# dkotfis/Octree-SLAM

Hardware: AMD Instinct MI355X
Metric: SLAM frames/sec (fuse+ICP+raycast) (higher is better)
Workload: dtype u32/f32 (ICP sums exact fixed-point in f64); 1 GPU; cfg3: synthetic 640x480 RGB-D stream, depth-12 SVO, half-edge 4.096 m, bilateral+ICP(19 it)+fuse+raycast(reference mode); parallelism=single GPU, frames_in_map_at_end=300, frames_input=resident in HBM

## Files before the change

### include/svoslam.h

```cpp
#ifndef SVOSLAM_H_
#define SVOSLAM_H_

#include <stddef.h>
#include <stdint.h>

#ifdef __cplusplus
extern "C" {
#endif

#define SVOSLAM_ABI_VERSION 1

typedef enum {
  SVOSLAM_OK = 0,
  SVOSLAM_ERR_INVALID_ARG = -1,
  SVOSLAM_ERR_NO_DEVICE = -2,
  SVOSLAM_ERR_HIP = -3,
  SVOSLAM_ERR_OOM = -4,
  SVOSLAM_ERR_DEPTH = -5,
  SVOSLAM_ERR_POOL_LIMIT = -6,
  SVOSLAM_ERR_TRACKING_LOST = -7,
  SVOSLAM_ERR_IO = -8,
  SVOSLAM_ERR_FORMAT = -9
} svoslam_status;

#define SVOSLAM_MAX_DEPTH 16
#define SVOSLAM_FLAG_CHILDREN 0x40000000u
#define SVOSLAM_CHILD_MASK 0x3FFFFFFFu

int svoslam_abi_version(void);
const char *svoslam_status_string(int status);

typedef struct svoslam_config {
  int32_t march_bricks;
  int32_t track_mode;
  int32_t track_workers;
  int32_t track_stream;
  int32_t runner_deferred;
  int32_t runner_lead;
  int32_t runner_prio;
  int32_t runner_replicas;
  int32_t runner_timeline;
  int32_t sort_pairs;
  int32_t graphs;
  int32_t march_ahead;
  int32_t reserved[4];
} svoslam_config;
int svoslam_config_get(svoslam_config *out);
int svoslam_config_set(const svoslam_config *in);
const char *svoslam_last_error(void);
const char *svoslam_device_arch(void);

typedef struct {
  uint32_t *d_data;
  int32_t size;
  int32_t capacity;
  int32_t *d_size;
  int32_t pending;
  int64_t pending_bound;
  void *tracker;
} svoslam_pool;

int svoslam_pool_init(svoslam_pool *pool, int32_t capacity_nodes, void *stream);
int svoslam_pool_reserve(svoslam_pool *pool, int32_t capacity_nodes, void *stream);
int svoslam_pool_free(svoslam_pool *pool);
int svoslam_pool_reset(svoslam_pool *pool, void *stream);
int svoslam_pool_sync(svoslam_pool *pool, void *stream);
int svoslam_pool_expand(svoslam_pool *pool, float center[3], float *edge_length, const float toward[3], void *stream);
int svoslam_pool_save(svoslam_pool *pool, const char *path, const float center[3], float edge_length, int32_t max_depth,
                      void *stream);
int svoslam_pool_touch(svoslam_pool *pool);
int svoslam_pool_march_accel(const svoslam_pool *pool, int32_t *has_grid, int32_t *brick_state, int32_t *brick_shift);
int svoslam_pool_set_nodes(svoslam_pool *pool, const uint32_t *h_words, int32_t num_nodes, void *stream);
int svoslam_pool_evict_subtree(svoslam_pool *pool, const uint8_t *path, int32_t levels, const char *file, void *stream);
int svoslam_pool_restore_subtree(svoslam_pool *pool, const char *file, void *stream);
int svoslam_subtree_file_nodes(const char *file, uint32_t **h_words, int32_t *num_nodes);
int svoslam_pool_graft_subtree(svoslam_pool *pool, const char *file, void *stream);
typedef struct {
  int32_t size_before, size_after;
  int32_t capacity_before, capacity_after;
  int32_t levels;
  int32_t tiles_dropped;
} svoslam_compact_stats;
int svoslam_pool_compact(svoslam_pool *pool, int32_t capacity_nodes, uint32_t *d_old_tile, svoslam_compact_stats *stats,
                         void *stream);
int svoslam_pool_copy(svoslam_pool *dst, svoslam_pool *src, void *stream);
int svoslam_pool_load(svoslam_pool *pool, const char *path, float center[3], float *edge_length, int32_t *max_depth,
                      void *stream);

typedef struct svoslam_workspace svoslam_workspace;
int svoslam_workspace_create(svoslam_workspace **ws);
int svoslam_workspace_destroy(svoslam_workspace *ws);

typedef struct {
  int32_t num_points;
  int32_t num_split;
  int32_t pass_sizes[SVOSLAM_MAX_DEPTH + 1];
  int32_t pool_size_before;
  int32_t pool_size_after;
} svoslam_fuse_stats;

int svoslam_svo_from_point_cloud(svoslam_workspace *ws, const float *d_points, const uint8_t *d_colors,
                                 int32_t n, int32_t max_depth, svoslam_pool *pool, const float center[3],
                                 float edge_length, svoslam_fuse_stats *stats, void *stream);

int svoslam_svo_from_point_cloud_async(svoslam_workspace *ws, const float *d_points, const uint8_t *d_colors,
                                       int32_t n, int32_t max_depth, svoslam_pool *pool, const float center[3],
                                       float edge_length, void *stream);

int svoslam_svo_fuse_sort(svoslam_workspace *ws, const float *d_points, int32_t n, int32_t max_depth,
                          const float center[3], float edge_length, void *stream);
int svoslam_svo_fuse_sort_frame(svoslam_workspace *ws, const uint16_t *d_depth, const float *d_pose, int32_t width, int32_t height,
                                float fx, float fy, int32_t max_depth, const float center[3], float edge_length, float *d_bbox7,
                                void *stream);
int svoslam_svo_fuse_plan(svoslam_workspace *ws, int32_t n, int32_t max_depth, svoslam_pool *pool, void *stream);
// ... 252 lines not shown
```

### octree-slam_amd/__init__.py

```python
import ctypes as C
import os

import numpy as np

_HERE = os.path.dirname(os.path.abspath(__file__))
LIB_PATH = os.path.join(_HERE, "libsvoslam_hip.so")
HEADER_PATH = os.path.join(os.path.dirname(_HERE), "include", "svoslam.h")

MAX_DEPTH = 16
FLAG_CHILDREN = 0x40000000
CHILD_MASK = 0x3FFFFFFF
RENDER_REFERENCE = 0
RENDER_CARRY = 1
PYRAMID_ITERS = (10, 5, 4)
DELTA_FLOATS = 20


class SvoslamError(RuntimeError):
    pass


def build(verbose=False, force=False):
    import importlib.util
    spec = importlib.util.spec_from_file_location("_svoslam_build", os.path.join(_HERE, "build.py"))
# ... 67 lines not shown
    "svoslam_svo_fuse_split_early": (C.c_int, [_vp, _i32, _i32, C.POINTER(_PoolStruct), _vp]),
    "svoslam_svo_fuse_plan_structure": (C.c_int, [_vp, _i32, _i32, C.POINTER(_PoolStruct), _vp]),
    "svoslam_svo_fuse_adopt_sorted": (C.c_int, [_vp, _vp, _vp, _i32, _i32]),
    "svoslam_svo_fuse_sort_frame_band": (C.c_int, [_vp, _vp, _vp, _i32, _i32, _f32, _f32, _i32, _fp, _f32, _i32, _i32, _vp]),
    "svoslam_svo_fuse_merge_sorted": (C.c_int, [C.POINTER(_vp), C.POINTER(_vp), C.POINTER(_i32), _i32, _vp, _vp, _vp]),
    "svoslam_svo_fuse_export_sorted": (C.c_int, [_vp, _i32, _vp, _vp, _vp]),
    "svoslam_pool_structure_begin": (C.c_int, [C.POINTER(_PoolStruct), _vp]),
    "svoslam_svo_fuse_commit_deferred": (C.c_int, [_vp, _vp, _i32, _i32, C.POINTER(_PoolStruct), _vp]),
    "svoslam_svo_fuse_apply": (C.c_int, [_vp, C.POINTER(_PoolStruct), _vp]),
    "svoslam_svo_fuse_keyrange_commit": (C.c_int, [_vp, _vp, _vp, _vp, _i32, _i32, C.POINTER(_PoolStruct), _i32, _i32, _vp, C.c_int64, _vp]),
    "svoslam_svo_fuse_keyrange_apply": (C.c_int, [_vp, _vp, _i32, _i32, C.POINTER(_PoolStruct), C.POINTER(C.c_void_p), _i32, _vp]),
    "svoslam_svo_fuse_keyrange_status": (C.c_int, [_vp, C.POINTER(C.c_int32), _vp]),
    "svoslam_svo_fuse_keyrange_discard": (C.c_int, [_vp, C.POINTER(_PoolStruct)]),
    "svoslam_frame_reader_open": (C.c_int, [C.POINTER(_vp), C.c_char_p, _f32]),
    "svoslam_frame_reader_close": (C.c_int, [_vp]),
    "svoslam_frame_reader_info": (C.c_int, [_vp, C.POINTER(_i32), C.POINTER(_i32), C.POINTER(_i32)]),
    "svoslam_frame_reader_rewind": (C.c_int, [_vp]),
    "svoslam_frame_reader_next_host": (C.c_int, [_vp, _vp, _vp, C.POINTER(C.c_longlong), C.POINTER(_i32)]),
    "svoslam_frame_reader_next": (C.c_int, [_vp, _vp, _vp, C.POINTER(C.c_longlong), C.POINTER(_i32), _vp]),
    "svoslam_focal_from_fov": (C.c_int, [_i32, _i32, _f32, _f32, _fp, _fp]),
    "svoslam_image_load": (C.c_int, [C.c_char_p, C.POINTER(_vp), C.POINTER(_i32), C.POINTER(_i32), C.POINTER(_i32), C.POINTER(_i32)]),
    "svoslam_workspace_create": (C.c_int, [C.POINTER(_vp)]),
    "svoslam_workspace_destroy": (C.c_int, [_vp]),
    "svoslam_svo_from_point_cloud": (C.c_int, [_vp, _vp, _vp, _i32, _i32, C.POINTER(_PoolStruct), _fp, _f32,
                                                C.POINTER(FuseStats), _vp]),
    "svoslam_svo_from_voxel_grid": (C.c_int, [_vp, _vp, _vp, _i32, _i32, C.POINTER(_PoolStruct), _fp, _f32,
                                               C.POINTER(FuseStats), _vp]),
    "svoslam_extract_voxel_grid": (C.c_int, [_vp, C.POINTER(_PoolStruct), _i32, _fp, _f32, C.POINTER(_vp),
                                              C.POINTER(_vp), C.POINTER(_i32), _vp]),
    "svoslam_mesh_load_obj": (C.c_int, [C.c_char_p, C.POINTER(MeshStruct)]),
    "svoslam_mesh_free": (C.c_int, [C.POINTER(MeshStruct)]),
    "svoslam_texture_load_bmp": (C.c_int, [C.c_char_p, C.POINTER(TextureStruct)]),
    "svoslam_texture_free": (C.c_int, [C.POINTER(TextureStruct)]),
    "svoslam_mesh_to_voxel_grid": (C.c_int, [_vp, C.POINTER(MeshStruct), C.POINTER(TextureStruct), _i32, _i32, C.POINTER(_vp),
                                             C.POINTER(_vp), C.POINTER(_vp), C.POINTER(_i32), _fp, _vp]),
    "svoslam_mesh_last_fragments": (C.c_int, [_vp, C.POINTER(C.c_int64)]),
    "svoslam_voxel_grid_to_mesh": (C.c_int, [_vp, _vp, _vp, _i32, _f32, _fp, _i32, C.POINTER(C.c_int32), _i32, _fp, _vp, _vp, _vp, _vp, _vp]),
    "svoslam_memcpy_h2d": (C.c_int, [_vp, _vp, C.c_size_t]),
    "svoslam_memcpy_d2h": (C.c_int, [_vp, _vp, C.c_size_t]),
    "svoslam_runner_run_model": (C.c_int, [_vp, C.POINTER(_vp), C.POINTER(_vp), C.POINTER(C.c_longlong), _fp, _i32, _vp, _i32, _i32, _vp,
                                           _f32, C.POINTER(_i32), _vp]),
    "svoslam_runner_create": (C.c_int, [C.POINTER(_vp), _vp, C.POINTER(_PoolStruct), _i32, _i32, _i32, _fp, _f32, _f32, _f32, _i32]),
    "svoslam_runner_destroy": (C.c_int, [_vp]),
    "svoslam_runner_timeline": (C.c_int, [_vp, _fp, _i32, C.POINTER(_i32)]),
    "svoslam_runner_run": (C.c_int, [_vp, C.POINTER(_vp), C.POINTER(_vp), C.POINTER(C.c_longlong), _fp, _i32, _vp, _i32, _i32, _vp, _vp]),
    "svoslam_runner_bbox": (C.c_int, [_vp, _fp]),
# ... 122 lines not shown


def _stream():
    global _raw_stream
    import torch
    if _raw_stream is None:
        _raw_stream = getattr(torch._C, "_cuda_getCurrentRawStream", None) or False
    if _raw_stream:
        return C.c_void_p(_raw_stream(torch.cuda.current_device()))
    return C.c_void_p(torch.cuda.current_stream().cuda_stream)


def _ptr(t):
    return C.c_void_p(t.data_ptr()) if t is not None else C.c_void_p(0)


def _fa(values, n):
    a = (C.c_float * n)(*[float(v) for v in np.asarray(values, dtype=np.float32).reshape(-1)])
    return a


class ConfigStruct(C.Structure):
    _fields_ = [(n, C.c_int32) for n in ("march_bricks", "track_mode", "track_workers", "track_stream", "runner_deferred", "runner_lead",
                                         "runner_prio", "runner_replicas", "runner_timeline", "sort_pairs", "graphs", "march_ahead")] + [("reserved", C.c_int32 * 4)]


def get_config():
    c = ConfigStruct()
    check(lib().svoslam_config_get(C.byref(c)))
    return {n: int(getattr(c, n)) for n, _ in ConfigStruct._fields_ if n != "reserved"}


def configure(**settings):
    c = ConfigStruct()
    check(lib().svoslam_config_get(C.byref(c)))
    before = {n: int(getattr(c, n)) for n, _ in ConfigStruct._fields_ if n != "reserved"}
    for k, v in settings.items():
        if k not in before:
            raise KeyError("svoslam_config has no field %r" % (k,))
        setattr(c, k, int(v))
    check(lib().svoslam_config_set(C.byref(c)))
    return before


def config_env(**settings):
    return {"SVOSLAM_CONFIG": ",".join("%s=%d" % (k, int(v)) for k, v in settings.items())}


def device_arch():
    a = lib().svoslam_device_arch()
    return a.decode() if a else None


class Workspace:
    def __init__(self):
        self._h = C.c_void_p()
        check(lib().svoslam_workspace_create(C.byref(self._h)))

    def close(self):
        if self._h:
            lib().svoslam_workspace_destroy(self._h)
            self._h = C.c_void_p()

    def __del__(self):
        try:
            self.close()
        except Exception:
            pass


class Pool:

    def __init__(self, capacity_nodes=8):
        self._p = _PoolStruct(None, 0, 0, None, 0, 0)
        check(lib().svoslam_pool_init(C.byref(self._p), capacity_nodes, _stream()))

    @property
    def size(self):
        if self._p.pending > 0:
            check(lib().svoslam_pool_sync(C.byref(self._p), _stream()))
        return int(self._p.size)

    @property
    def capacity(self):
        return int(self._p.capacity)
# ... 932 lines not shown
```

### octree-slam_amd/csrc/abi.hip

```cpp
#include <stdarg.h>
#include <stdio.h>
#include <string.h>

#include "common.hpp"
#include "cone_trace.hpp"
#include "icp.hpp"
#include "image_kernels.hpp"
#include "map_query.hpp"
#include "mesh.hpp"
#include "model_depth.hpp"
#include "frame_io.hpp"
#include "pool_grid.hpp"
#include "stage_timing.hpp"
#include "svo_build.hpp"
#include "workspace.hpp"

namespace svoslam {

static thread_local char g_last_error[512] = "";
static char g_arch[256] = "";
static int g_device_state = 0;

void set_last_error_text(const char *fmt, ...) {
  va_list ap;
// ... 279 lines not shown
  void *p = malloc(img.data.size() ? img.data.size() : 1);
  if (!p) return SVOSLAM_ERR_OOM;
  memcpy(p, img.data.data(), img.data.size());
  *h_data = p;
  if (width) *width = img.width;
  if (height) *height = img.height;
  if (channels) *channels = img.channels;
  if (bits) *bits = img.bits;
  return SVOSLAM_OK;
}

int svoslam_workspace_create(svoslam_workspace **ws) {
  if (!ws) return SVOSLAM_ERR_INVALID_ARG;
  NEED_DEVICE();
  *ws = new svoslam_workspace();
  return SVOSLAM_OK;
}
int svoslam_workspace_destroy(svoslam_workspace *ws) {
  if (!ws) return SVOSLAM_OK;
  ws->release_all();
  delete ws;
  return SVOSLAM_OK;
}

int svoslam_svo_from_point_cloud(svoslam_workspace *ws, const float *d_points, const uint8_t *d_colors, int32_t n,
                                 int32_t max_depth, svoslam_pool *pool, const float center[3], float edge_length,
                                 svoslam_fuse_stats *stats, void *stream) {
  NEED_DEVICE();
  if (!center) return SVOSLAM_ERR_INVALID_ARG;
  return svo_from_point_cloud(ws, d_points, d_colors, n, max_depth, pool, center, edge_length, stats, S(stream));
}

int svoslam_svo_from_voxel_grid(svoslam_workspace *ws, const float *d_centers, const float *d_colors, int32_t n,
                                int32_t max_depth, svoslam_pool *pool, const float center[3], float edge_length,
                                svoslam_fuse_stats *stats, void *stream) {
  NEED_DEVICE();
  if (!center) return SVOSLAM_ERR_INVALID_ARG;
  return svo_from_voxel_grid(ws, d_centers, d_colors, n, max_depth, pool, center, edge_length, stats, S(stream));
}

int svoslam_extract_voxel_grid(svoslam_workspace *ws, const svoslam_pool *pool, int32_t max_depth, const float center[3],
                               float edge_length, float **d_centers, float **d_colors, int32_t *n_out, void *stream) {
  NEED_DEVICE();
  if (!center) return SVOSLAM_ERR_INVALID_ARG;
  return extract_voxel_grid(ws, pool, max_depth, center, edge_length, d_centers, d_colors, n_out, S(stream));
}
// ... 311 lines not shown
```

### octree-slam_amd/csrc/config.hip

```cpp
#include <cstdio>
#include <cstdlib>
#include <cstring>
#include <mutex>

#include "config.hpp"

namespace svoslam {
namespace {
std::mutex g_mu;
bool g_ready = false;
svoslam_config g_cfg;

struct Field { const char *name; int32_t svoslam_config::*member; };
const Field kFields[] = {
    {"march_bricks", &svoslam_config::march_bricks}, {"track_mode", &svoslam_config::track_mode},
    {"track_workers", &svoslam_config::track_workers}, {"track_stream", &svoslam_config::track_stream},
    {"runner_deferred", &svoslam_config::runner_deferred}, {"runner_lead", &svoslam_config::runner_lead},
    {"runner_prio", &svoslam_config::runner_prio}, {"runner_replicas", &svoslam_config::runner_replicas},
    {"runner_timeline", &svoslam_config::runner_timeline}, {"sort_pairs", &svoslam_config::sort_pairs},
    {"graphs", &svoslam_config::graphs}, {"march_ahead", &svoslam_config::march_ahead},
};

bool config_valid(const svoslam_config &c) {
  if (c.runner_replicas != 1 || c.graphs != 0) return false;
  if (c.track_mode < 0 || c.track_mode > 2 || c.track_workers < 0) return false;
  return true;
}

void init_locked() {
  if (g_ready) return;
  memset(&g_cfg, 0, sizeof(g_cfg));
  g_cfg.march_bricks = 1; g_cfg.track_stream = 1; g_cfg.march_ahead = 60;
  g_cfg.runner_deferred = -1; g_cfg.runner_lead = -1; g_cfg.runner_prio = -1; g_cfg.runner_replicas = 1;
  if (const char *e = getenv("SVOSLAM_CONFIG")) {
    const char *p = e;
    while (*p) {
      const char *eq = strchr(p, '='), *end = strchr(p, ',');
      if (!end) end = p + strlen(p);
      bool known = false;
      if (eq && eq < end && eq > p) {
        for (const Field &f : kFields)
          if ((size_t)(eq - p) == strlen(f.name) && strncmp(p, f.name, (size_t)(eq - p)) == 0) {
            known = true;
            svoslam_config trial = g_cfg;
            char *stop = nullptr;
            const long v = strtol(eq + 1, &stop, 10);
            trial.*(f.member) = (int32_t)v;
            if (stop == eq + 1 || stop != end || !config_valid(trial))
              fprintf(stderr, "svoslam: SVOSLAM_CONFIG: value of '%s' rejected (\"%.*s\"); the default stays\n", f.name, (int)(end - p), p);
            else
              g_cfg = trial;
          }
      }
      if (!known && end > p) fprintf(stderr, "svoslam: SVOSLAM_CONFIG: unknown or malformed entry \"%.*s\" ignored\n", (int)(end - p), p);
      p = *end ? end + 1 : end;
// ... 29 lines not shown
```

### octree-slam_amd/csrc/svo_build.hip

```cpp
#include <stdlib.h>
#include <string.h>

#include <cstdio>
#include <vector>

#include "radix_sort.hpp"
#include "image_device.hpp"
#include "config.hpp"
#include "pool_grid.hpp"
#include "svo_build.hpp"
#include "svo_fuse_internal.hpp"
#include "stage_timing.hpp"
#include "wave_rank.hpp"

namespace svoslam {

constexpr unsigned char kNotHead = 0xFE;
constexpr unsigned char kNoSplit = 0xFF;

template <int STRIDE>
__global__ __launch_bounds__(256) void compute_keys_kernel(const float *__restrict__ pts, int n, int depth, float cx,
                                                           float cy, float cz, float edge, u64 *__restrict__ keys, int idx_bits = -1) {
  const int i = blockIdx.x * 256 + threadIdx.x;
  if (i >= n) return;
// ... 463 lines not shown
__device__ inline void shadow_store(unsigned long long *__restrict__ shadow, u32 epoch, u32 node, u32 word) {
  shadow[node] = ((unsigned long long)epoch << 32) | word;
}

__global__ __launch_bounds__(256) void mip_level_kernel(int n, int d, const unsigned char *__restrict__ leaf_c,
                                                        const u32 *__restrict__ path_nodes, u32 *__restrict__ pool) {
  const long long j0 = ((long long)blockIdx.x * 256 + threadIdx.x) * 4;
  if (j0 >= n) return;
  u32 c4 = 0xFFFFFFFFu;
  if (j0 + 3 < n) c4 = *reinterpret_cast<const u32 *>(leaf_c + j0);
  else for (int k = 0; k < 4 && j0 + k < n; k++) c4 = (c4 & ~(0xFFu << (8 * k))) | ((u32)leaf_c[j0 + k] << (8 * k));
#pragma unroll
  for (int k = 0; k < 4; k++) {
    if ((int)((c4 >> (8 * k)) & 0xFFu) >= d) continue;
    const u32 node = path_nodes[(size_t)(d - 1) * n + (size_t)(j0 + k)];
    pool[2 * (size_t)node + 1] = average_tile(pool, pool[2 * (size_t)node] & kMask);
  }
}

__global__ void mip_root_kernel(u32 *__restrict__ pool, const PlanCounts *__restrict__ counts) {
  if (threadIdx.x == 0 && blockIdx.x == 0 && counts->any_valid) pool[1] = average_tile(pool, 0);
}

template <int MAXD>
__global__ __launch_bounds__(kFillThreads) void fill_mip_local_kernel(const u64 *__restrict__ skey, const u32 *__restrict__ sidx, int n,
                                                             int depth, const unsigned char *__restrict__ leaf_t,
                                                             const unsigned char *__restrict__ colors, u32 *__restrict__ pool,
                                                             u32 *__restrict__ strad, int num_tiles, u32 *__restrict__ grid_dirty,
                                                             unsigned long long *__restrict__ shadow, u32 epoch,
                                                             u32 *__restrict__ apply_nodes, const u64 *__restrict__ rec_key,
                                                             const u32 *__restrict__ bucket_base, const u32 *__restrict__ n0_saved,
                                                             const u32 *__restrict__ leaf_rec0, const u32 *__restrict__ leaf_start,
                                                             int *__restrict__ strad_bc, int brick_shift, const int *__restrict__ n_live) {
  if (n_live) { const int nl = *n_live; n = nl < n ? nl : n; }
  const bool early_links = leaf_rec0 != nullptr;
  SVO_HIGH_PRIO();
  __shared__ int last_owner[SVOSLAM_MAX_DEPTH + 1];
  __shared__ int next_pos, next_c;
  __shared__ int min_c;
  __shared__ u32 apply_cnt;
  const int tid = (int)threadIdx.x;
  const int bid = xcd_tile(num_tiles);
  if (bid >= num_tiles) return;
  int search_tiles = num_tiles;
  if (n_live) {
    const int live_tiles = (n + kFillThreads - 1) / kFillThreads;
    if (bid >= live_tiles) {
      if (tid >= 1 && tid < depth) {
        strad[2 * ((size_t)tid * num_tiles + bid)] = kNoStraddler;
        strad[2 * ((size_t)tid * num_tiles + bid) + 1] = 0u;
      }
      if (shadow && tid == 0) apply_nodes[(size_t)num_tiles * kFillThreads * (size_t)depth + bid] = 0u;
      return;
    }
    search_tiles = live_tiles;
  }
  if (tid == 0) apply_cnt = 0;
  u32 *apply_mine = apply_nodes ? apply_nodes + (size_t)bid * kFillThreads * (size_t)depth : nullptr;
  auto apply_append = [&](bool mine, u32 node) {
    const unsigned long long m = __ballot(mine);
    if (!m) return;
    u32 base = 0;
    if ((tid & 63) == 0) base = atomicAdd(&apply_cnt, (u32)__popcll(m));
    base = (u32)__shfl((int)base, 0);
    if (mine) apply_mine[base + (u32)__popcll(m & lanemask_lt())] = node;
  };
  const int j = bid * kFillThreads + tid;
  const int jn = j + kFillThreads;
  const unsigned char lt = j < n ? leaf_t[j] : kNotHead;
  const unsigned char ltn = jn < n ? leaf_t[jn] : kNotHead;
  const u64 key_j = j < n ? skey[j] : 1ull, key_p = (j > 0 && j < n) ? skey[j - 1] : 1ull;
  const u64 key_n = jn < n ? skey[jn] : 1ull, key_np = jn < n ? skey[jn - 1] : 1ull;
  const u32 point = j < n ? sidx[j] : 0u;
  const bool head = lt != kNotHead;
  const u32 start_base = (leaf_start && head) ? leaf_start[j] : 0u;
  u32 rec0 = 0;
  if (early_links && head && lt != kNoSplit) {
    const int cc = (key_p == 1ull) ? 0 : common_levels(key_j, key_p, depth);
    if (cc < (int)lt) rec0 = leaf_rec0[j];
  }
  u64 key = 1; int c = 0;
  if (head) { key = key_j; c = (key_p == 1ull) ? 0 : common_levels(key_j, key_p, depth); }
  if (grid_dirty && head && c < kPoolGridBlockLevel) pool_grid_mark(grid_dirty, key, depth);
  __shared__ u32 brick_cnt, brick_base;
  const bool bricks_on = grid_dirty != nullptr && brick_shift >= 0 && depth >= brick_node_level(brick_shift);
  u32 brick_entry = 0, brick_off = 0;
  const bool brick_mine = bricks_on && brick_mark_test(grid_dirty, head && c < brick_node_level(brick_shift), key, depth, brick_shift, brick_entry);
  if (tid <= SVOSLAM_MAX_DEPTH) {
    last_owner[tid] = -1;
    if (tid >= 1 && tid < depth) {
      strad[2 * ((size_t)tid * num_tiles + bid)] = kNoStraddler;
      strad[2 * ((size_t)tid * num_tiles + bid) + 1] = 0u;
    }
  }
  if (tid == 0) { next_pos = 0x7FFFFFFF; next_c = -1; min_c = 99; brick_cnt = 0u; }
  __syncthreads();
  if (bricks_on) {
    const unsigned long long bm = __ballot(brick_mine);
    if (bm) {
      const int leader = __ffsll((long long)bm) - 1;
      u32 woff = 0;
      if ((tid & 63) == leader) woff = atomicAdd(&brick_cnt, (u32)__popcll(bm));
      brick_off = (u32)__shfl((int)woff, leader) + (u32)__popcll(bm & ((1ull << (tid & 63)) - 1ull));
    }
  }
  if (head) {
    for (int d = c + 1; d < depth; d++) atomicMax(&last_owner[d], j);
    if (strad_bc) atomicMin(&min_c, c);
  }
  if (ltn != kNotHead) atomicMin(&next_pos, jn);
  __syncthreads();
  if (bricks_on && tid == 0 && brick_cnt) brick_base = brick_ring_reserve(grid_dirty, brick_cnt);
  if (next_pos == 0x7FFFFFFF) {
    for (int nb = bid + 2; nb < search_tiles; nb++) {
      const int jj = nb * kFillThreads + tid;
      if (jj < n && leaf_t[jj] != kNotHead) atomicMin(&next_pos, jj);
      __syncthreads();
      const bool found = next_pos != 0x7FFFFFFF;
      __syncthreads();
      if (found) break;
    }
    if (tid == 0 && next_pos != 0x7FFFFFFF) {
      u64 k2; int c2 = 0;
      (void)is_head(skey, next_pos, k2, c2, depth);
      next_c = c2;
    }
  } else if (jn == next_pos) {
    next_c = (key_np == 1ull) ? 0 : common_levels(key_n, key_np, depth);
  }
  if (strad_bc) {
    __syncthreads();
    if (tid == 0) { strad_bc[2 * bid] = next_c; strad_bc[2 * bid + 1] = min_c; }
  }
  int frontier = 0;
  int link_level = 0;
  u32 frontier_child = 0;
  bool have_rec0 = false;
  if (early_links) {
    __shared__ u32 wave_rec0[kFillThreads / 64];
    __shared__ int wave_has[kFillThreads / 64];
    const bool towner = head && lt != kNoSplit && c < (int)lt;
    const unsigned lane = (unsigned)tid & 63u, wv = (unsigned)tid >> 6;
    const unsigned long long om = __ballot(towner);
    const unsigned long long upto = om & ((lane == 63u) ? ~0ull : ((2ull << lane) - 1ull));
    const int src = upto ? 63 - __clzll((long long)upto) : -1;
    const u32 got = (u32)__shfl((int)rec0, src >= 0 ? src : 0);
    const int last = om ? 63 - __clzll((long long)om) : 0;
    const u32 lastv = (u32)__shfl((int)rec0, last);
    if (lane == 0) { wave_has[wv] = om != 0ull; wave_rec0[wv] = lastv; }
    __syncthreads();
    if (src >= 0) { rec0 = got; have_rec0 = true; }
    else {
      for (int w = (int)wv - 1; w >= 0; w--)
        if (wave_has[w]) { rec0 = wave_rec0[w]; have_rec0 = true; break; }
    }
// ... 24 lines not shown
  if (head) {
    const unsigned char *v = colors + 3 * (size_t)point;
    const unsigned char cr = v[0], cg = v[1], cb = v[2];
    int skip = 0;
    u32 base = 0, node = 0;
    if (leaf_start) {
      const int tt = lt == kNoSplit ? depth : (int)lt - 1;
      skip = c < tt ? c : tt;
      base = start_base;
    }
#pragma unroll
    for (int lvl = 1; lvl <= MAXD; lvl++) {
      if (lvl <= depth && lvl > skip) {
        node = base + ((u32)(key >> (3 * (depth - lvl))) & 7u);
        if (lvl == link_level) pool[2 * (size_t)node] = kFlag + (frontier_child & kMask);
        if (lvl < depth) {
          base = pool[2 * (size_t)node] & kMask;
          if (lvl == frontier) base = frontier_child & kMask;
          node_at[lvl] = node;
          child_at[lvl] = base;
        }
      }
    }
    const u32 word = blend_color256(pool[2 * (size_t)node + 1], cr, cg, cb);
    if (shadow) shadow_store(shadow, epoch, node, word);
    else pool[2 * (size_t)node + 1] = word;
    node_at[0] = node;
  }
  if (shadow) apply_append(head, node_at[0]);
  __syncthreads();
  if (brick_mine) brick_ring_store(grid_dirty, brick_base + brick_off, brick_entry);
#pragma unroll
  for (int d = MAXD - 1; d >= 1; d--) {
    if (d < depth) {
      u32 wrote = kNoStraddler;
      if (head && c < d) {
        if (j != last_owner[d] || next_c < d) {
          if (shadow) {
            shadow_store(shadow, epoch, node_at[d], average_tile_deferred(pool, shadow, epoch, child_at[d]));
            wrote = node_at[d];
          } else {
            pool[2 * (size_t)node_at[d] + 1] = average_tile(pool, child_at[d]);
          }
        } else {
          strad[2 * ((size_t)d * num_tiles + bid)] = node_at[d];
          strad[2 * ((size_t)d * num_tiles + bid) + 1] = child_at[d];
        }
      }
      if (shadow) apply_append(wrote != kNoStraddler, wrote);
      __syncthreads();
    }
  }
  if (brick_mine && lt != kNoSplit && (int)lt < brick_node_level(brick_shift)) brick_sibling_list(grid_dirty, brick_entry);
  if (shadow && tid == 0) apply_nodes[(size_t)num_tiles * kFillThreads * (size_t)depth + bid] = apply_cnt;
}

constexpr int kStradThreads = 1024;
__global__ __launch_bounds__(kStradThreads) void mip_straddle_kernel(u32 *__restrict__ pool, const u32 *__restrict__ strad, int num_tiles,
                                                            int depth, const PlanCounts *__restrict__ counts,
                                                            int *__restrict__ d_size, u32 *__restrict__ grid_dirty,
                                                            int32_t *__restrict__ h_sizes, int *__restrict__ d_slot,
                                                            unsigned long long *__restrict__ shadow, u32 epoch, int keep_size,
                                                            const int *__restrict__ n_live) {
  SVO_HIGH_PRIO();
  const int list_stride = num_tiles;
  if (n_live) { const int live = (*n_live + kFillThreads - 1) / kFillThreads; num_tiles = live < num_tiles ? live : num_tiles; }
  auto average = [&](u32 child_base) { return shadow ? average_tile_deferred(pool, shadow, epoch, child_base) : average_tile(pool, child_base); };
  auto store = [&](u32 node, u32 word) {
    if (shadow) shadow_store(shadow, epoch, node, word);
    else pool[2 * (size_t)node + 1] = word;
  };
  constexpr int kSlots = 8;
  const uint2 *list = reinterpret_cast<const uint2 *>(strad);
  const bool fits = num_tiles <= kSlots * kStradThreads;
  uint2 cur[kSlots], nxt[kSlots];
  auto fetch = [&](int d, uint2 *e) {
#pragma unroll
// ... 14 lines not shown
    } else {
      for (int t = (int)threadIdx.x; t < num_tiles; t += kStradThreads) {
        const uint2 e = list[(size_t)d * list_stride + t];
        if (e.x != kNoStraddler) store(e.x, average(e.y));
      }
    }
    __syncthreads();
  }
  if (threadIdx.x == 0) {
    if (counts->any_valid) store(0u, average(0u));
    if (!keep_size) {
      const int size_now = *d_size + 8 * counts->total_records;
      *d_size = size_now;
      if (h_sizes) {
        const int sl = *d_slot;
        h_sizes[sl] = size_now;
        *d_slot = (sl + 1) % 8;
      }
    }
  }
  if (grid_dirty) pool_grid_compact(grid_dirty, kStradThreads);
}

constexpr int kStradGroup = 16;
constexpr int kStrad2Threads = 256;
__global__ __launch_bounds__(kStrad2Threads) void mip_straddle2_kernel(u32 *__restrict__ pool, const u32 *__restrict__ strad,
                                                              const int *__restrict__ strad_bc, u32 *__restrict__ sstrad,
                                                              unsigned *__restrict__ ticket, int num_tiles, int depth,
                                                              const PlanCounts *__restrict__ counts, int *__restrict__ d_size,
                                                              u32 *__restrict__ grid_dirty, int32_t *__restrict__ h_sizes,
                                                              int *__restrict__ d_slot) {
  SVO_HIGH_PRIO();
  __shared__ int bc[kStradGroup], mc[kStradGroup];
  __shared__ int is_last;
  const int tid = (int)threadIdx.x, g = (int)blockIdx.x, groups = (int)gridDim.x;
  const int t0 = g * kStradGroup, t1 = (t0 + kStradGroup < num_tiles) ? t0 + kStradGroup : num_tiles;
  const uint2 *list = reinterpret_cast<const uint2 *>(strad);
  uint2 *super = reinterpret_cast<uint2 *>(sstrad);
  if (tid < kStradGroup) {
    bc[tid] = (t0 + tid < t1) ? strad_bc[2 * (t0 + tid)] : -1;
    mc[tid] = (t0 + tid < t1) ? strad_bc[2 * (t0 + tid) + 1] : 99;
  }
  __syncthreads();
  const int t = t0 + tid;
  for (int d = depth - 1; d >= 1; d--) {
    if (tid < kStradGroup) {
      uint2 sup = make_uint2(kNoStraddler, 0u);
// ... 469 lines not shown
    return SVOSLAM_OK;
  }
  const int64_t rmax = max_records(n, depth);
  if (pool != ws->planned_pool) {
    SVO_TRY(ensure_device_size(pool, stream));
    if ((int64_t)pool->size + pool->pending_bound + 8 * rmax > pool->capacity) {
      SVO_TRY(tracker_poll(pool, true));
      if ((int64_t)pool->size + pool->pending_bound + 8 * rmax > pool->capacity) return SVOSLAM_ERR_POOL_LIMIT;
    }
    pool->pending_bound += 8 * rmax;
  }
  const u64 *skey = ws->sorted_keys;
  const u32 *sidx = ws->sorted_idx;
  const unsigned char *leaf_t = ws->leaf_t.as<unsigned char>();
  int split_blocks = (int)cdiv(rmax, 256);
  if (split_blocks > 2048) split_blocks = 2048;
  const int fill_tiles = (int)cdiv(n, kFillThreads);
  const int strad_groups = (int)cdiv(fill_tiles, kStradGroup);
  const size_t strad_words = (size_t)(SVOSLAM_MAX_DEPTH + 1) * (size_t)fill_tiles * 2, bc_words = 2 * (size_t)fill_tiles;
  SVO_TRY(ws->strad.reserve((strad_words + bc_words + (size_t)(SVOSLAM_MAX_DEPTH + 1) * (size_t)strad_groups * 2) * 4));
  u32 *strad = ws->strad.as<u32>();
  int *strad_bc = reinterpret_cast<int *>(strad + strad_words);
  u32 *sstrad = strad + strad_words + bc_words;
  const bool two_tier = !deferred;
  const u32 *leaf_start = ws->leaf_start.as<u32>();
  SVO_TRY(ensure_device_size(pool, stream));
  PoolTracker *trk = tracker_of(pool);
  unsigned long long *shadow = nullptr;
  u32 epoch = 0, *apply_nodes = nullptr;
  if (deferred) {
    SVO_TRY(ws->apply_nodes.reserve(((size_t)fill_tiles * kFillThreads * (size_t)depth + (size_t)fill_tiles) * 4));
    apply_nodes = ws->apply_nodes.as<u32>();
    SVO_TRY(pool_shadow_begin(pool, stream, &shadow, &epoch));
    ws->deferred_pool = pool; ws->deferred_n = n; ws->deferred_depth = depth; ws->deferred_tiles = fill_tiles;
  }
  SVO_TRY(tracker_make_room(pool));
  int brick_shift = -1;
  u32 *grid_dirty = keyrange ? nullptr : pool_accel_dirty_bitmap(pool, deferred ? (int)(epoch & 1u) : 0, depth, &brick_shift);
  {
    StageScope timed(kStageFuseCommit, stream);
    if (!early)
      split_all_kernel<<<split_blocks, 256, 0, stream>>>(ws->rec_key.as<u64>(), ws->rec_front.as<u32>(),
                                                         ws->rec_pass.as<unsigned char>(), small_bucket_base(ws), small_counts(ws),
                                                         pool->d_data, pool->d_size, depth, grid_dirty, deferred ? small_n0(ws) : nullptr, 0);
    if (depth <= 12) fill_mip_local_kernel<12><<<xcd_grid(fill_tiles), kFillThreads, 0, stream>>>(skey, sidx, n, depth, leaf_t, d_colors, pool->d_data, strad, fill_tiles,
                                                                   grid_dirty, shadow, epoch, apply_nodes, ws->rec_key.as<u64>(),
                                                                   small_bucket_base(ws), small_n0(ws), early ? ws->leaf_rec0.as<u32>() : nullptr, leaf_start,
                                                                   two_tier ? strad_bc : nullptr, brick_shift, n_live);
    else fill_mip_local_kernel<16><<<xcd_grid(fill_tiles), kFillThreads, 0, stream>>>(skey, sidx, n, depth, leaf_t, d_colors, pool->d_data, strad, fill_tiles,
                                                                   grid_dirty, shadow, epoch, apply_nodes, ws->rec_key.as<u64>(),
                                                                   small_bucket_base(ws), small_n0(ws), early ? ws->leaf_rec0.as<u32>() : nullptr, leaf_start,
                                                                   two_tier ? strad_bc : nullptr, brick_shift, n_live);
    if (two_tier)
      mip_straddle2_kernel<<<strad_groups, kStrad2Threads, 0, stream>>>(pool->d_data, strad, strad_bc, sstrad, small_strad_ticket(ws), fill_tiles,
                                                                        depth, small_counts(ws), pool->d_size, grid_dirty,
                                                                        trk ? trk->h_size : nullptr, trk ? trk->d_slot : nullptr);
    else
      mip_straddle_kernel<<<1, kStradThreads, 0, stream>>>(pool->d_data, strad, fill_tiles, depth, small_counts(ws), pool->d_size, grid_dirty,
                                                           trk ? trk->h_size : nullptr, trk ? trk->d_slot : nullptr, shadow, epoch, keyrange ? 1 : 0, n_live);
    SVO_LAUNCH_CHECK();
  }
  if (keyrange) { ws->keyrange_bound = 8 * rmax; return SVOSLAM_OK; }
  pool->pending += 1;
  return tracker_push(pool, 8 * rmax, stream);
}

int svo_fuse_commit(svoslam_workspace *ws, const uint8_t *d_colors, int n, int depth, svoslam_pool *pool, hipStream_t stream) {
  return commit_impl(ws, d_colors, n, depth, pool, false, stream);
}

int svo_fuse_commit_deferred(svoslam_workspace *ws, const uint8_t *d_colors, int n, int depth, svoslam_pool *pool, hipStream_t stream) {
  return commit_impl(ws, d_colors, n, depth, pool, true, stream);
}

int svo_fuse_apply(svoslam_workspace *ws, svoslam_pool *pool, hipStream_t stream) {
  if (!ws || !pool || ws->deferred_pool != pool) return SVOSLAM_ERR_INVALID_ARG;
  ws->deferred_pool = nullptr;
  const int n = ws->deferred_n, depth = ws->deferred_depth, tiles = ws->deferred_tiles;
  if (n == 0) return SVOSLAM_OK;
  unsigned long long *shadow = nullptr;
  u32 epoch = 0;
  SVO_TRY(pool_shadow_current(pool, &shadow, &epoch));
// ... 57 lines not shown
```

### octree-slam_amd/csrc/workspace.hpp

```cpp
#pragma once

#include "common.hpp"

namespace svoslam {

struct DeviceBuffer {
  void *ptr = nullptr;
  size_t bytes = 0;
  int reserve(size_t need) {
    if (need <= bytes) return SVOSLAM_OK;
    if (ptr) { SVO_HIP(hipFree(ptr)); ptr = nullptr; bytes = 0; }
    size_t want = need + need / 4 + 256;
    SVO_HIP(hipMalloc(&ptr, want));
    bytes = want;
    return SVOSLAM_OK;
  }
  void release() {
    if (ptr) (void)hipFree(ptr);
    ptr = nullptr; bytes = 0;
  }
  template <class T> T *as() const { return reinterpret_cast<T *>(ptr); }
};

struct PlanCounts {
  int32_t total_records;
  int32_t pass_start[SVOSLAM_MAX_DEPTH + 2];
  int32_t any_valid;
};

}

struct svoslam_workspace {
  svoslam::DeviceBuffer keys_a, keys_b, vals_a, vals_b;
  svoslam::DeviceBuffer tile_hist;
  svoslam::DeviceBuffer small;
  svoslam::DeviceBuffer leaf_t, leaf_f;
  svoslam::DeviceBuffer rec_key, rec_front;
  svoslam::DeviceBuffer rec_pass;
  svoslam::DeviceBuffer leaf_rec0;
  svoslam::DeviceBuffer leaf_start;
  svoslam::DeviceBuffer path_nodes;
  svoslam::DeviceBuffer strad;
  svoslam::DeviceBuffer kr_keys, kr_idx, kr_small;
  const void *keyrange_pool = nullptr;
  svoslam::DeviceBuffer apply_nodes;
  const void *deferred_pool = nullptr;
  int deferred_n = 0, deferred_depth = 0, deferred_tiles = 0;
  svoslam::DeviceBuffer bfs_a, bfs_b, bfs_mask, bfs_ptr;
  svoslam::DeviceBuffer surf_color, surf_tiles;
  svoslam::DeviceBuffer misc;
  svoslam::DeviceBuffer scan_tmp;
  svoslam::DeviceBuffer frame_bbox;
  svoslam::PlanCounts *h_counts = nullptr;
  long long mesh_fragments = 0;
  const unsigned long long *sorted_keys = nullptr;
  const unsigned int *sorted_idx = nullptr;
  int planned_n = -1;
  const void *early_split_pool = nullptr;
  bool structure_planned = false;
  long long keyrange_bound = 0;
  const void *planned_pool = nullptr;
  unsigned int planned_numbering = 0;
  int reserve_small() {
    if (small.bytes >= 4096) return SVOSLAM_OK;
    SVO_TRY(small.reserve(4096));
    SVO_HIP(svoslam::memset_sync(small.ptr, 0, small.bytes));
    return SVOSLAM_OK;
  }
  void release_all() {
    keys_a.release(); keys_b.release(); vals_a.release(); vals_b.release(); tile_hist.release(); small.release();
    leaf_t.release(); leaf_f.release(); rec_key.release(); rec_front.release(); path_nodes.release(); strad.release();
    rec_pass.release(); apply_nodes.release(); leaf_rec0.release(); leaf_start.release();
    kr_keys.release(); kr_idx.release(); kr_small.release();
    bfs_a.release(); bfs_b.release(); bfs_mask.release(); bfs_ptr.release(); surf_color.release(); surf_tiles.release(); misc.release(); scan_tmp.release(); frame_bbox.release();
    if (h_counts) { (void)hipHostFree(h_counts); h_counts = nullptr; }
  }
};
```

Baseline: 2604 frames/s.

## Fuse straddler mip resolution into fill kernel via last-block ticket tiers

Adds a commit_tiers mode, on by default, that folds the separate straddle-resolution kernel into the tail of the fill/mip kernel. A two-level ticket scheme makes the last block of each 16-tile group resolve that group's straddlers, and the last group finalize the super-level straddlers, the root colour and the pool size. This removes one kernel launch and the dependency gap between fill and straddle per commit. In exchange, stores are now agent-scope atomics with extra fences, the work runs on a single block tail, and a persistent ticket buffer is added along with a debug accessor for it.

```diff
diff --git a/include/svoslam.h b/include/svoslam.h
--- a/include/svoslam.h
+++ b/include/svoslam.h
@@ -43,7 +43,8 @@
   int32_t sort_pairs;
   int32_t graphs;
   int32_t march_ahead;
-  int32_t reserved[4];
+  int32_t commit_tiers;
+  int32_t reserved[3];
 } svoslam_config;
 int svoslam_config_get(svoslam_config *out);
 int svoslam_config_set(const svoslam_config *in);
@@ -90,6 +91,7 @@
 typedef struct svoslam_workspace svoslam_workspace;
 int svoslam_workspace_create(svoslam_workspace **ws);
 int svoslam_workspace_destroy(svoslam_workspace *ws);
+int svoslam_workspace_commit_tickets(svoslam_workspace *ws, uint32_t *h_words, int32_t capacity, int32_t *count);
 
 typedef struct {
   int32_t num_points;
diff --git a/octree-slam_amd/__init__.py b/octree-slam_amd/__init__.py
--- a/octree-slam_amd/__init__.py
+++ b/octree-slam_amd/__init__.py
@@ -113,6 +113,7 @@
     "svoslam_image_load": (C.c_int, [C.c_char_p, C.POINTER(_vp), C.POINTER(_i32), C.POINTER(_i32), C.POINTER(_i32), C.POINTER(_i32)]),
     "svoslam_workspace_create": (C.c_int, [C.POINTER(_vp)]),
     "svoslam_workspace_destroy": (C.c_int, [_vp]),
+    "svoslam_workspace_commit_tickets": (C.c_int, [_vp, C.POINTER(C.c_uint32), C.c_int32, C.POINTER(C.c_int32)]),
     "svoslam_svo_from_point_cloud": (C.c_int, [_vp, _vp, _vp, _i32, _i32, C.POINTER(_PoolStruct), _fp, _f32,
                                                 C.POINTER(FuseStats), _vp]),
     "svoslam_svo_from_voxel_grid": (C.c_int, [_vp, _vp, _vp, _i32, _i32, C.POINTER(_PoolStruct), _fp, _f32,
@@ -281,7 +282,8 @@
 
 class ConfigStruct(C.Structure):
     _fields_ = [(n, C.c_int32) for n in ("march_bricks", "track_mode", "track_workers", "track_stream", "runner_deferred", "runner_lead",
-                                         "runner_prio", "runner_replicas", "runner_timeline", "sort_pairs", "graphs", "march_ahead")] + [("reserved", C.c_int32 * 4)]
+                                         "runner_prio", "runner_replicas", "runner_timeline", "sort_pairs", "graphs", "march_ahead",
+                                         "commit_tiers")] + [("reserved", C.c_int32 * 3)]
 
 
 def get_config():
@@ -320,6 +322,13 @@
         if self._h:
             lib().svoslam_workspace_destroy(self._h)
             self._h = C.c_void_p()
+
+    def commit_tickets(self):
+        n = C.c_int32(0)
+        check(lib().svoslam_workspace_commit_tickets(self._h, None, 0, C.byref(n)))
+        out = np.zeros(max(int(n.value), 1), np.uint32)
+        check(lib().svoslam_workspace_commit_tickets(self._h, out.ctypes.data_as(C.POINTER(C.c_uint32)), int(n.value), C.byref(n)))
+        return out[: int(n.value)]
 
     def __del__(self):
         try:
diff --git a/octree-slam_amd/csrc/abi.hip b/octree-slam_amd/csrc/abi.hip
--- a/octree-slam_amd/csrc/abi.hip
+++ b/octree-slam_amd/csrc/abi.hip
@@ -325,6 +325,16 @@
   delete ws;
   return SVOSLAM_OK;
 }
+int svoslam_workspace_commit_tickets(svoslam_workspace *ws, uint32_t *h_words, int32_t capacity, int32_t *count) {
+  if (!ws || !count || capacity < 0 || (capacity > 0 && !h_words)) return SVOSLAM_ERR_INVALID_ARG;
+  NEED_DEVICE();
+  const size_t have = ws->commit_tickets.bytes / 4;
+  *count = (int32_t)have;
+  const size_t take = have < (size_t)capacity ? have : (size_t)capacity;
+  SVO_HIP(hipDeviceSynchronize());
+  if (take) SVO_HIP(hipMemcpy(h_words, ws->commit_tickets.ptr, take * 4, hipMemcpyDeviceToHost));
+  return SVOSLAM_OK;
+}
 
 int svoslam_svo_from_point_cloud(svoslam_workspace *ws, const float *d_points, const uint8_t *d_colors, int32_t n,
                                  int32_t max_depth, svoslam_pool *pool, const float center[3], float edge_length,
diff --git a/octree-slam_amd/csrc/config.hip b/octree-slam_amd/csrc/config.hip
--- a/octree-slam_amd/csrc/config.hip
+++ b/octree-slam_amd/csrc/config.hip
@@ -19,18 +19,20 @@
     {"runner_prio", &svoslam_config::runner_prio}, {"runner_replicas", &svoslam_config::runner_replicas},
     {"runner_timeline", &svoslam_config::runner_timeline}, {"sort_pairs", &svoslam_config::sort_pairs},
     {"graphs", &svoslam_config::graphs}, {"march_ahead", &svoslam_config::march_ahead},
+    {"commit_tiers", &svoslam_config::commit_tiers},
 };
 
 bool config_valid(const svoslam_config &c) {
   if (c.runner_replicas != 1 || c.graphs != 0) return false;
   if (c.track_mode < 0 || c.track_mode > 2 || c.track_workers < 0) return false;
+  if (c.commit_tiers < 0 || c.commit_tiers > 1) return false;
   return true;
 }
 
 void init_locked() {
   if (g_ready) return;
   memset(&g_cfg, 0, sizeof(g_cfg));
-  g_cfg.march_bricks = 1; g_cfg.track_stream = 1; g_cfg.march_ahead = 60;
+  g_cfg.march_bricks = 1; g_cfg.track_stream = 1; g_cfg.march_ahead = 60; g_cfg.commit_tiers = 1;
   g_cfg.runner_deferred = -1; g_cfg.runner_lead = -1; g_cfg.runner_prio = -1; g_cfg.runner_replicas = 1;
   if (const char *e = getenv("SVOSLAM_CONFIG")) {
     const char *p = e;
diff --git a/octree-slam_amd/csrc/svo_build.hip b/octree-slam_amd/csrc/svo_build.hip
--- a/octree-slam_amd/csrc/svo_build.hip
+++ b/octree-slam_amd/csrc/svo_build.hip
@@ -509,7 +509,13 @@
   if (threadIdx.x == 0 && blockIdx.x == 0 && counts->any_valid) pool[1] = average_tile(pool, 0);
 }
 
-template <int MAXD>
+constexpr int kStradGroup = 16;
+__device__ inline void commit_tiers_finish(u32 *__restrict__ pool, u32 *__restrict__ strad, int *__restrict__ strad_bc, u32 *__restrict__ sstrad,
+                                           unsigned *__restrict__ tickets, int num_tiles, int bid, int depth,
+                                           const PlanCounts *__restrict__ counts, int *__restrict__ d_size, u32 *__restrict__ grid_dirty,
+                                           int32_t *__restrict__ h_sizes, int *__restrict__ d_slot, unsigned long long *__restrict__ shadow,
+                                           u32 epoch);
+template <int MAXD, bool TIERS>
 __global__ __launch_bounds__(kFillThreads) void fill_mip_local_kernel(const u64 *__restrict__ skey, const u32 *__restrict__ sidx, int n,
                                                              int depth, const unsigned char *__restrict__ leaf_t,
                                                              const unsigned char *__restrict__ colors, u32 *__restrict__ pool,
@@ -518,7 +524,10 @@
                                                              u32 *__restrict__ apply_nodes, const u64 *__restrict__ rec_key,
                                                              const u32 *__restrict__ bucket_base, const u32 *__restrict__ n0_saved,
                                                              const u32 *__restrict__ leaf_rec0, const u32 *__restrict__ leaf_start,
-                                                             int *__restrict__ strad_bc, int brick_shift, const int *__restrict__ n_live) {
+                                                             int *__restrict__ strad_bc, int brick_shift, const int *__restrict__ n_live,
+                                                             u32 *__restrict__ sstrad, unsigned *__restrict__ tickets,
+                                                             const PlanCounts *__restrict__ counts, int *__restrict__ d_size,
+                                                             int32_t *__restrict__ h_sizes, int *__restrict__ d_slot) {
   if (n_live) { const int nl = *n_live; n = nl < n ? nl : n; }
   const bool early_links = leaf_rec0 != nullptr;
   SVO_HIGH_PRIO();
@@ -552,6 +561,21 @@
     base = (u32)__shfl((int)base, 0);
     if (mine) apply_mine[base + (u32)__popcll(m & lanemask_lt())] = node;
   };
+  auto put_word = [&](u32 node, u32 word) {
+    if (shadow) {
+      if (TIERS) __hip_atomic_store(shadow + node, ((unsigned long long)epoch << 32) | word, __ATOMIC_RELAXED, __HIP_MEMORY_SCOPE_AGENT);
+      else shadow_store(shadow, epoch, node, word);
+    } else {
+      if (TIERS) __hip_atomic_store(&pool[2 * (size_t)node + 1], word, __ATOMIC_RELAXED, __HIP_MEMORY_SCOPE_AGENT);
+      else pool[2 * (size_t)node + 1] = word;
+    }
+  };
+  auto put_strad = [&](int d, u32 node, u32 child) {
+    u32 *e = strad + 2 * ((size_t)d * num_tiles + bid);
+    if (TIERS) {
+      __hip_atomic_store(reinterpret_cast<unsigned long long *>(e), ((unsigned long long)child << 32) | node, __ATOMIC_RELAXED, __HIP_MEMORY_SCOPE_AGENT);
+    } else { e[0] = node; e[1] = child; }
+  };
   const int j = bid * kFillThreads + tid;
   const int jn = j + kFillThreads;
   const unsigned char lt = j < n ? leaf_t[j] : kNotHead;
@@ -575,10 +599,7 @@
   const bool brick_mine = bricks_on && brick_mark_test(grid_dirty, head && c < brick_node_level(brick_shift), key, depth, brick_shift, brick_entry);
   if (tid <= SVOSLAM_MAX_DEPTH) {
     last_owner[tid] = -1;
-    if (tid >= 1 && tid < depth) {
-      strad[2 * ((size_t)tid * num_tiles + bid)] = kNoStraddler;
-      strad[2 * ((size_t)tid * num_tiles + bid) + 1] = 0u;
-    }
+    if (tid >= 1 && tid < depth) put_strad(tid, kNoStraddler, 0u);
   }
   if (tid == 0) { next_pos = 0x7FFFFFFF; next_c = -1; min_c = 99; brick_cnt = 0u; }
   __syncthreads();
@@ -617,7 +638,12 @@
   }
   if (strad_bc) {
     __syncthreads();
-    if (tid == 0) { strad_bc[2 * bid] = next_c; strad_bc[2 * bid + 1] = min_c; }
+    if (tid == 0) {
+      if (TIERS) {
+        __hip_atomic_store(&strad_bc[2 * bid], next_c, __ATOMIC_RELAXED, __HIP_MEMORY_SCOPE_AGENT);
+        __hip_atomic_store(&strad_bc[2 * bid + 1], min_c, __ATOMIC_RELAXED, __HIP_MEMORY_SCOPE_AGENT);
+      } else { strad_bc[2 * bid] = next_c; strad_bc[2 * bid + 1] = min_c; }
+    }
   }
   int frontier = 0;
   int link_level = 0;
@@ -688,9 +714,7 @@
         }
       }
     }
-    const u32 word = blend_color256(pool[2 * (size_t)node + 1], cr, cg, cb);
-    if (shadow) shadow_store(shadow, epoch, node, word);
-    else pool[2 * (size_t)node + 1] = word;
+    put_word(node, blend_color256(pool[2 * (size_t)node + 1], cr, cg, cb));
     node_at[0] = node;
   }
   if (shadow) apply_append(head, node_at[0]);
@@ -703,14 +727,13 @@
       if (head && c < d) {
         if (j != last_owner[d] || next_c < d) {
           if (shadow) {
-            shadow_store(shadow, epoch, node_at[d], average_tile_deferred(pool, shadow, epoch, child_at[d]));
+            put_word(node_at[d], average_tile_deferred(pool, shadow, epoch, child_at[d]));
             wrote = node_at[d];
           } else {
-            pool[2 * (size_t)node_at[d] + 1] = average_tile(pool, child_at[d]);
+            put_word(node_at[d], average_tile(pool, child_at[d]));
           }
         } else {
-          strad[2 * ((size_t)d * num_tiles + bid)] = node_at[d];
-          strad[2 * ((size_t)d * num_tiles + bid) + 1] = child_at[d];
+          put_strad(d, node_at[d], child_at[d]);
         }
       }
       if (shadow) apply_append(wrote != kNoStraddler, wrote);
@@ -719,6 +742,123 @@
   }
   if (brick_mine && lt != kNoSplit && (int)lt < brick_node_level(brick_shift)) brick_sibling_list(grid_dirty, brick_entry);
   if (shadow && tid == 0) apply_nodes[(size_t)num_tiles * kFillThreads * (size_t)depth + bid] = apply_cnt;
+  if (TIERS) commit_tiers_finish(pool, strad, strad_bc, sstrad, tickets, num_tiles, bid, depth, counts, d_size, grid_dirty, h_sizes, d_slot, shadow, epoch);
+}
+
+typedef __attribute__((address_space(1))) unsigned long long tier_gu64;
+typedef __attribute__((address_space(1))) u32 tier_gu32;
+__device__ __noinline__ void tier_finish_node(u32 *pool, unsigned long long *shadow, u32 epoch, u32 node, u32 child_base) {
+  tier_gu64 *tile = (tier_gu64 *)(pool + 2 * (size_t)child_base);
+  u32 w[8];
+#pragma unroll
+  for (int q = 0; q < 8; q++) w[q] = (u32)(__hip_atomic_load(tile + q, __ATOMIC_RELAXED, __HIP_MEMORY_SCOPE_AGENT) >> 32);
+  if (shadow) {
+    tier_gu64 *sh = (tier_gu64 *)(shadow + child_base);
+#pragma unroll
+    for (int q = 0; q < 8; q++) {
+      const unsigned long long t = __hip_atomic_load(sh + q, __ATOMIC_RELAXED, __HIP_MEMORY_SCOPE_AGENT);
+      if ((u32)(t >> 32) == epoch) w[q] = (u32)t;
+    }
+  }
+  u32 r = 0, g = 0, b = 0, a = 0;
+#pragma unroll
+  for (int q = 0; q < 8; q++) {
+    r += w[q] & 0xFF; g += (w[q] >> 8) & 0xFF; b += (w[q] >> 16) & 0xFF;
+    const u32 aa = w[q] >> 24;
+    a = a > aa ? a : aa;
+  }
+  const u32 word = (r >> 3) + ((g >> 3) << 8) + ((b >> 3) << 16) + (a << 24);
+  if (shadow) __hip_atomic_store((tier_gu64 *)(shadow + node), ((unsigned long long)epoch << 32) | word, __ATOMIC_RELAXED, __HIP_MEMORY_SCOPE_AGENT);
+  else __hip_atomic_store((tier_gu32 *)(pool + 2 * (size_t)node + 1), word, __ATOMIC_RELAXED, __HIP_MEMORY_SCOPE_AGENT);
+}
+
+__device__ inline void commit_tiers_finish(u32 *__restrict__ pool, u32 *__restrict__ strad, int *__restrict__ strad_bc, u32 *__restrict__ sstrad,
+                                           unsigned *__restrict__ tickets, int num_tiles, int bid, int depth,
+                                           const PlanCounts *__restrict__ counts, int *__restrict__ d_size, u32 *__restrict__ grid_dirty,
+                                           int32_t *__restrict__ h_sizes, int *__restrict__ d_slot, unsigned long long *__restrict__ shadow,
+                                           u32 epoch) {
+  __shared__ int bc[kStradGroup], mc[kStradGroup];
+  __shared__ int is_last;
+  const int tid = (int)threadIdx.x;
+  const int groups = (num_tiles + kStradGroup - 1) / kStradGroup, g = bid / kStradGroup;
+  const int t0 = g * kStradGroup, t1 = (t0 + kStradGroup < num_tiles) ? t0 + kStradGroup : num_tiles;
+  unsigned long long *list = reinterpret_cast<unsigned long long *>(strad);
+  unsigned long long *super = reinterpret_cast<unsigned long long *>(sstrad);
+  auto finish = [&](u32 node, u32 child_base) { tier_finish_node(pool, shadow, epoch, node, child_base); };
+  asm volatile("s_waitcnt vmcnt(0)" ::: "memory");
+  __syncthreads();
+  if (tid == 0) {
+    const unsigned k = __hip_atomic_fetch_add(tickets + 1 + g, 1u, __ATOMIC_RELAXED, __HIP_MEMORY_SCOPE_AGENT);
+    is_last = k == (unsigned)(t1 - t0) - 1u;
+  }
+  __syncthreads();
+  if (!is_last) return;
+  if (tid == 0) {
+    __builtin_amdgcn_fence(__ATOMIC_ACQUIRE, "agent");
+    __hip_atomic_store(tickets + 1 + g, 0u, __ATOMIC_RELAXED, __HIP_MEMORY_SCOPE_AGENT);
+  }
+  if (tid < kStradGroup) {
+    bc[tid] = (t0 + tid < t1) ? __hip_atomic_load(&strad_bc[2 * (t0 + tid)], __ATOMIC_RELAXED, __HIP_MEMORY_SCOPE_AGENT) : -1;
+    mc[tid] = (t0 + tid < t1) ? __hip_atomic_load(&strad_bc[2 * (t0 + tid) + 1], __ATOMIC_RELAXED, __HIP_MEMORY_SCOPE_AGENT) : 99;
+  }
+  asm volatile("s_waitcnt vmcnt(0)" ::: "memory");
+  __syncthreads();
+  const int t = t0 + tid;
+  for (int d = depth - 1; d >= 1; d--) {
+    if (tid < kStradGroup) {
+      unsigned long long sup = kNoStraddler;
+      if (t < t1) {
+        const unsigned long long e = __hip_atomic_load(&list[(size_t)d * num_tiles + t], __ATOMIC_RELAXED, __HIP_MEMORY_SCOPE_AGENT);
+        if ((u32)e != kNoStraddler) {
+          bool inside = false;
+          for (int b = tid + 1; b < t1 - t0; b++)
+            if (mc[b] < d || bc[b] < d) { inside = true; break; }
+          if (inside) finish((u32)e, (u32)(e >> 32));
+          else sup = e;
+        }
+      }
+      const unsigned long long m = __ballot((u32)sup != kNoStraddler);
+      if (m) {
+        const int src = __ffsll((long long)m) - 1;
+        const u32 lo = (u32)__shfl((int)(u32)sup, src), hi = (u32)__shfl((int)(u32)(sup >> 32), src);
+        sup = ((unsigned long long)hi << 32) | lo;
+      }
+      if (tid == 0) __hip_atomic_store(&super[(size_t)d * groups + g], sup, __ATOMIC_RELAXED, __HIP_MEMORY_SCOPE_AGENT);
+    }
+    asm volatile("s_waitcnt vmcnt(0)" ::: "memory");
+    __syncthreads();
+  }
+  if (tid == 0) {
+    const unsigned k = __hip_atomic_fetch_add(tickets, 1u, __ATOMIC_RELAXED, __HIP_MEMORY_SCOPE_AGENT);
+    is_last = k == (unsigned)groups - 1u;
+  }
+  __syncthreads();
+  if (!is_last) return;
+  if (tid == 0) {
+    __builtin_amdgcn_fence(__ATOMIC_ACQUIRE, "agent");
+    __hip_atomic_store(tickets, 0u, __ATOMIC_RELAXED, __HIP_MEMORY_SCOPE_AGENT);
+  }
+  asm volatile("s_waitcnt vmcnt(0)" ::: "memory");
+  __syncthreads();
+  for (int d = depth - 1; d >= 1; d--) {
+    for (int q = tid; q < groups; q += kFillThreads) {
+      const unsigned long long e = __hip_atomic_load(&super[(size_t)d * groups + q], __ATOMIC_RELAXED, __HIP_MEMORY_SCOPE_AGENT);
+      if ((u32)e != kNoStraddler) finish((u32)e, (u32)(e >> 32));
+    }
+    asm volatile("s_waitcnt vmcnt(0)" ::: "memory");
+    __syncthreads();
+  }
+  if (tid == 0) {
+    if (counts->any_valid) finish(0u, 0u);
+    const int size_now = *d_size + 8 * counts->total_records;
+    *d_size = size_now;
+    if (h_sizes) {
+      const int sl = *d_slot;
+      h_sizes[sl] = size_now;
+      *d_slot = (sl + 1) % 8;
+    }
+  }
+  if (grid_dirty) pool_grid_compact(grid_dirty, kFillThreads);
 }
 
 constexpr int kStradThreads = 1024;
@@ -779,7 +919,6 @@
   if (grid_dirty) pool_grid_compact(grid_dirty, kStradThreads);
 }
 
-constexpr int kStradGroup = 16;
 constexpr int kStrad2Threads = 256;
 __global__ __launch_bounds__(kStrad2Threads) void mip_straddle2_kernel(u32 *__restrict__ pool, const u32 *__restrict__ strad,
                                                               const int *__restrict__ strad_bc, u32 *__restrict__ sstrad,
@@ -1295,7 +1434,10 @@
   u32 *strad = ws->strad.as<u32>();
   int *strad_bc = reinterpret_cast<int *>(strad + strad_words);
   u32 *sstrad = strad + strad_words + bc_words;
-  const bool two_tier = !deferred;
+  const bool tiers = !keyrange && config().commit_tiers != 0;
+  const bool two_tier = !deferred && !tiers;
+  if (tiers) SVO_TRY(ws->reserve_commit_tickets((size_t)strad_groups));
+  unsigned *tickets = tiers ? ws->commit_tickets.as<unsigned>() : nullptr;
   const u32 *leaf_start = ws->leaf_start.as<u32>();
   SVO_TRY(ensure_device_size(pool, stream));
   PoolTracker *trk = tracker_of(pool);
@@ -1316,21 +1458,28 @@
       split_all_kernel<<<split_blocks, 256, 0, stream>>>(ws->rec_key.as<u64>(), ws->rec_front.as<u32>(),
                                                          ws->rec_pass.as<unsigned char>(), small_bucket_base(ws), small_counts(ws),
                                                          pool->d_data, pool->d_size, depth, grid_dirty, deferred ? small_n0(ws) : nullptr, 0);
-    if (depth <= 12) fill_mip_local_kernel<12><<<xcd_grid(fill_tiles), kFillThreads, 0, stream>>>(skey, sidx, n, depth, leaf_t, d_colors, pool->d_data, strad, fill_tiles,
-                                                                   grid_dirty, shadow, epoch, apply_nodes, ws->rec_key.as<u64>(),
-                                                                   small_bucket_base(ws), small_n0(ws), early ? ws->leaf_rec0.as<u32>() : nullptr, leaf_start,
-                                                                   two_tier ? strad_bc : nullptr, brick_shift, n_live);
-    else fill_mip_local_kernel<16><<<xcd_grid(fill_tiles), kFillThreads, 0, stream>>>(skey, sidx, n, depth, leaf_t, d_colors, pool->d_data, strad, fill_tiles,
-                                                                   grid_dirty, shadow, epoch, apply_nodes, ws->rec_key.as<u64>(),
-                                                                   small_bucket_base(ws), small_n0(ws), early ? ws->leaf_rec0.as<u32>() : nullptr, leaf_start,
-                                                                   two_tier ? strad_bc : nullptr, brick_shift, n_live);
-    if (two_tier)
-      mip_straddle2_kernel<<<strad_groups, kStrad2Threads, 0, stream>>>(pool->d_data, strad, strad_bc, sstrad, small_strad_ticket(ws), fill_tiles,
-                                                                        depth, small_counts(ws), pool->d_size, grid_dirty,
-                                                                        trk ? trk->h_size : nullptr, trk ? trk->d_slot : nullptr);
-    else
-      mip_straddle_kernel<<<1, kStradThreads, 0, stream>>>(pool->d_data, strad, fill_tiles, depth, small_counts(ws), pool->d_size, grid_dirty,
-                                                           trk ? trk->h_size : nullptr, trk ? trk->d_slot : nullptr, shadow, epoch, keyrange ? 1 : 0, n_live);
+    int32_t *h_sizes = trk ? trk->h_size : nullptr;
+    int *d_slot = trk ? trk->d_slot : nullptr;
+#define SVO_FILL_LAUNCH(MAXD, TIERS)                                                                                                      \
+  fill_mip_local_kernel<MAXD, TIERS><<<xcd_grid(fill_tiles), kFillThreads, 0, stream>>>(                                                  \
+      skey, sidx, n, depth, leaf_t, d_colors, pool->d_data, strad, fill_tiles, grid_dirty, shadow, epoch, apply_nodes,                    \
+      ws->rec_key.as<u64>(), small_bucket_base(ws), small_n0(ws), early ? ws->leaf_rec0.as<u32>() : nullptr, leaf_start,                  \
+      (two_tier || tiers) ? strad_bc : nullptr, brick_shift, n_live, sstrad, tickets, small_counts(ws), pool->d_size, h_sizes, d_slot)
+    if (tiers) {
+      if (depth <= 12) SVO_FILL_LAUNCH(12, true);
+      else if (depth <= 14) SVO_FILL_LAUNCH(14, true);
+      else SVO_FILL_LAUNCH(16, true);
+    } else {
+      if (depth <= 12) SVO_FILL_LAUNCH(12, false);
+      else SVO_FILL_LAUNCH(16, false);
+      if (two_tier)
+        mip_straddle2_kernel<<<strad_groups, kStrad2Threads, 0, stream>>>(pool->d_data, strad, strad_bc, sstrad, small_strad_ticket(ws), fill_tiles,
+                                                                          depth, small_counts(ws), pool->d_size, grid_dirty, h_sizes, d_slot);
+      else
+        mip_straddle_kernel<<<1, kStradThreads, 0, stream>>>(pool->d_data, strad, fill_tiles, depth, small_counts(ws), pool->d_size, grid_dirty,
+                                                             h_sizes, d_slot, shadow, epoch, keyrange ? 1 : 0, n_live);
+    }
+#undef SVO_FILL_LAUNCH
     SVO_LAUNCH_CHECK();
   }
   if (keyrange) { ws->keyrange_bound = 8 * rmax; return SVOSLAM_OK; }
diff --git a/octree-slam_amd/csrc/workspace.hpp b/octree-slam_amd/csrc/workspace.hpp
--- a/octree-slam_amd/csrc/workspace.hpp
+++ b/octree-slam_amd/csrc/workspace.hpp
@@ -41,6 +41,7 @@
   svoslam::DeviceBuffer leaf_start;
   svoslam::DeviceBuffer path_nodes;
   svoslam::DeviceBuffer strad;
+  svoslam::DeviceBuffer commit_tickets;
   svoslam::DeviceBuffer kr_keys, kr_idx, kr_small;
   const void *keyrange_pool = nullptr;
   svoslam::DeviceBuffer apply_nodes;
@@ -67,7 +68,15 @@
     SVO_HIP(svoslam::memset_sync(small.ptr, 0, small.bytes));
     return SVOSLAM_OK;
   }
+  int reserve_commit_tickets(size_t groups) {
+    const size_t need = (groups + 1) * 4;
+    if (need <= commit_tickets.bytes) return SVOSLAM_OK;
+    SVO_TRY(commit_tickets.reserve(need));
+    SVO_HIP(svoslam::memset_sync(commit_tickets.ptr, 0, commit_tickets.bytes));
+    return SVOSLAM_OK;
+  }
   void release_all() {
+    commit_tickets.release();
     keys_a.release(); keys_b.release(); vals_a.release(); vals_b.release(); tile_hist.release(); small.release();
     leaf_t.release(); leaf_f.release(); rec_key.release(); rec_front.release(); path_nodes.release(); strad.release();
     rec_pass.release(); apply_nodes.release(); leaf_rec0.release(); leaf_start.release();
```

New measurement: 2431 frames/s. 6.6% lower.
